# zhoubin-me/agent0

Hardware: AMD Instinct MI355X
Metric: env-frames/sec (learner FPS: transitions collected and saved to replay per second with the learner running, pre-frameskip) (higher is better)
Workload: dtype f32

## Files before the change

agent0_amd/csrc/igemm_x9.h:

```cpp
#pragma once
#include "igemm.h"
#if defined(__HIPCC__)
#include <hip/hip_ext.h>
#endif

#if defined(__HIPCC__)

typedef __bf16 a0_bf16x8g __attribute__((ext_vector_type(8)));
typedef short a0_s16x4 __attribute__((ext_vector_type(4)));
typedef uint32_t a0_u32x2g __attribute__((ext_vector_type(2)));
typedef uint32_t a0_u32x4g __attribute__((ext_vector_type(4)));

struct a0_x9_piece {
    a0_f4 v;
    uint32_t h[4], m[4], l[4];
    A0_D void split(int e) {
        const float x = e == 0 ? v.x : e == 1 ? v.y : e == 2 ? v.z : v.w;
        h[e] = __float_as_uint(x);
        const float r1 = x - __uint_as_float(h[e] & 0xffff0000u);
        m[e] = __float_as_uint(r1);
        const float r2 = r1 - __uint_as_float(m[e] & 0xffff0000u);
        l[e] = __float_as_uint(r2);
    }
    A0_D void pack(a0_u32x2g& hi, a0_u32x2g& mid, a0_u32x2g& lo) const {
// ... 119 lines not shown
        return v;
    }
};
template <int BX, int NTH, int KS> struct a0_x9_stager<OpPlanesKC, BX, NTH, KS, A0_KC> {
    static constexpr bool PRESPLIT = true;
    static constexpr int TPR = 4 * KS;
    static constexpr int RPP = NTH / TPR;
    static constexpr int R = BX / RPP;
    static_assert(BX % RPP == 0, "tile rows per pass");
    typedef a0_x9_image<A0_KC, BX, KS> IM;
    typedef OpPlanesKC OP;
    OP::Row rows[R];
    OP::KInfo ki;
    struct Slot { OP::Raw raw[R]; unsigned okmask; };
    A0_D void init(const OP::Params& P, int x0, int X, int kb, int ke, int tid) {
#pragma unroll
        for (int j = 0; j < R; ++j) rows[j] = OP::row(P, x0 + tid / TPR + RPP * j, X);
        ki = OP::kinfo(P, kb + 4 * (tid % TPR), ke);
    }
    template <bool FULL = false> A0_D void fetch_piece(const OP::Params& P, Slot& s, int j, int k0, int ke, int tid) {
        s.raw[j] = OP::load(P, rows[j], ki);
        if (j == R - 1) ki = OP::kinfo(P, k0 + 16 * KS + 4 * (tid % TPR), ke);
    }
    template <bool RS, bool FULL = false> A0_D a0_f4 value(const Slot&, int, a0_f4&) const { return a0_zero4(); }
    A0_D void store(const a0_x9_piece&, int, char*, int) const {}
    A0_D void store_raw(const Slot& s, int j, char* lds, int tid) const {
        const int r = tid / TPR + RPP * j;
        char* p = lds + r * IM::PITCH + 8 * (tid % TPR);
        a0_u32x2g hi, mid; hi.x = s.raw[j].a.x; hi.y = s.raw[j].a.y; mid.x = s.raw[j].a.z; mid.y = s.raw[j].a.w;
        *(a0_u32x2g*)(p) = hi;
        *(a0_u32x2g*)(p + IM::PLANE) = mid;
        *(a0_u32x2g*)(p + 2 * IM::PLANE) = s.raw[j].b;
    }
    A0_D static int frag_base(int lane, int woff) { return (woff + (lane & 31)) * IM::PITCH + (lane >> 5) * 16; }
    A0_D static a0_u32x4g frag(const char* plane, int base, int blk, int s) {
        return *(const a0_u32x4g*)(plane + base + blk * 32 * IM::PITCH + s * 32);
    }
};

template <class OA, class OB, int WM, int WN, int MT, int NT, int KS = 2> struct a0_x9_geom {
    static constexpr int BX = WM * MT * 32, BY = WN * NT * 32;
    static constexpr int ABYTES = 3 * a0_x9_image<OA::MODE, BX, KS>::PLANE;
    static constexpr int BBYTES = 3 * a0_x9_image<OB::MODE, BY, KS>::PLANE;
    static constexpr int LDS_BYTES = 2 * (ABYTES + BBYTES);
};

template <class OP> struct a0_x9_plain { static constexpr bool value = false; };
template <> struct a0_x9_plain<OpMatKC> { static constexpr bool value = true; };
template <> struct a0_x9_plain<OpMatXC> { static constexpr bool value = true; };
struct OpPlanesKC;
template <> struct a0_x9_plain<OpPlanesKC> { static constexpr bool value = true; };
template <class EP> struct a0_is_hadamard { static constexpr bool value = false; };
template <> struct a0_is_hadamard<EpiHadamard> { static constexpr bool value = true; };

int a0_x9_products_now();
template <class OA, class OB, class EP, int WM, int WN, int MT, int NT, int KS = 2, int NPR = 9, bool FULL = false>
__device__ __forceinline__ void a0_igemm_x9_body(const typename OA::Params& pa, const typename OB::Params& pb,
                                                 const typename EP::Params& pe, int X, int Y, int K, int kchunk, int gx, int gy) {
    static_assert(WM * WN == 4 || WM * WN == 8, "four or eight waves per workgroup");
    static_assert(KS == 1 || KS == 2, "tiles of 16 or 32 k");
    typedef a0_x9_geom<OA, OB, WM, WN, MT, NT, KS> G;
    constexpr int BK = 16 * KS, BX = G::BX, BY = G::BY, NTH = WM * WN * 64;
    typedef a0_x9_stager<OA, BX, NTH, KS> SA;
    typedef a0_x9_stager<OB, BY, NTH, KS> SB;
    constexpr int APL = a0_x9_image<OA::MODE, BX, KS>::PLANE, BPL = a0_x9_image<OB::MODE, BY, KS>::PLANE;
    constexpr int RA = SA::R, RB = SB::R, NP = RA + RB;
    static_assert(NPR == 9 || NPR == 6, "nine or six cross products");
    constexpr int NG = NPR * KS;
    static_assert(!EP::ROWSUM_A || OA::MODE == A0_XC, "row sums need an x-contiguous A operand");
    extern __shared__ __attribute__((aligned(16))) char a0_x9_lds[];
    char* const As = a0_x9_lds;
    char* const Bs = a0_x9_lds + 2 * G::ABYTES;

    const int tid = threadIdx.x, lane = tid & 63, wave = tid >> 6;
    const int wm = wave / WN, wn = wave % WN;
    int bx, by, bz;
    {
        const int n = gridDim.x, id = blockIdx.x, per = n >> 3;
        const int L = (id < (per << 3)) ? (id & 7) * per + (id >> 3) : id;
        if (gy <= gx) { by = L % gy; const int t = L / gy; bx = t % gx; bz = t / gx; }
        else          { bx = L % gx; const int t = L / gx; by = t % gy; bz = t / gy; }
    }
    const int x0 = bx * BX, y0 = by * BY;
    const int kb = bz * kchunk;
    const int ke = (K < kb + kchunk) ? K : (kb + kchunk);

    SA sa; SB sb;
    sa.init(pa, x0, X, kb, ke, tid);
    sb.init(pb, y0, Y, kb, ke, tid);

    a0_acc16 acc[MT][NT];
#pragma unroll
    for (int i = 0; i < MT; ++i)
#pragma unroll
        for (int j = 0; j < NT; ++j)
#pragma unroll
            for (int r = 0; r < 16; ++r) acc[i][j][r] = 0.f;

    a0_f4 rowsum = a0_zero4();

    auto fetch_piece = [&](typename SA::Slot& s_a, typename SB::Slot& s_b, int p, int k0) {
        if (p < RA) sa.template fetch_piece<FULL>(pa, s_a, p, k0, ke, tid);
        else sb.template fetch_piece<FULL>(pb, s_b, p - RA, k0, ke, tid);
    };
    a0_x9_piece pc;
    auto micro = [&](int u, const typename SA::Slot& s_a_c, const typename SB::Slot& s_b_c, typename SA::Slot& s_a, typename SB::Slot& s_b,
// ... 70 lines not shown
        __syncthreads();
    }
    if constexpr (EP::ROWSUM_A) {
        if (by == 0) {
            constexpr int Q = BX / 4;
            a0_f4* red = (a0_f4*)a0_x9_lds;
            red[tid] = rowsum;
            __syncthreads();
            if (tid < BX && x0 + tid < X) {
                const float* rf = (const float*)a0_x9_lds;
                float t = 0.f;
#pragma unroll
                for (int g = 0; g < NTH / Q; ++g) t += rf[4 * (g * Q + (tid >> 2)) + (tid & 3)];
                EP::store_rowsum(pe, x0 + tid, t, bz);
            }
        }
    }

    if constexpr (a0_is_hadamard<EP>::value) {
        static_assert(MT == 2, "EpiHadamard: waves of 64 rows");
#pragma unroll
        for (int j = 0; j < NT; ++j) {
            const int y = y0 + wn * (NT * 32) + j * 32 + (lane & 31);
            const bool yok = y < Y;
            const int yy = yok ? y : 0;
            float s64 = 0.f;
#pragma unroll
            for (int i = 0; i < MT; ++i) {
                const int xb = x0 + wm * (MT * 32) + i * 32;
                const int bsmp = xb / pe.n;
                const float f = pe.feat[(long long)bsmp * pe.ld + yy];
                float sacc = 0.f;
                float ev[16];
#pragma unroll
                for (int r = 0; r < 16; ++r) ev[r] = pe.emb[(long long)(xb + (r & 3) + 8 * (r >> 2) + 4 * (lane >> 5)) * pe.ld + yy];
#pragma unroll
                for (int r = 0; r < 16; ++r) {
                    const long long idx = (long long)(xb + (r & 3) + 8 * (r >> 2) + 4 * (lane >> 5)) * pe.ld + yy;
                    const float g = acc[i][j][r];
                    if (yok) pe.demb[idx] = (ev[r] > 0.f) ? g * f : 0.f;
                    sacc += g * ev[r];
                }
                sacc += __shfl_xor(sacc, 32, 64);
                if (pe.n == 32) { if (yok && lane < 32) pe.d3[(long long)bsmp * pe.ld + y] = (f > 0.f) ? sacc : 0.f; }
                else {
                    s64 += sacc;
                    if (i == MT - 1 && yok && lane < 32) pe.d3[(long long)bsmp * pe.ld + y] = (f > 0.f) ? s64 : 0.f;
                }
            }
        }
        return;
    }
    const int z = bz;
#pragma unroll
    for (int i = 0; i < MT; ++i)
#pragma unroll
        for (int j = 0; j < NT; ++j) {
            const int y = y0 + wn * (NT * 32) + j * 32 + (lane & 31);
#pragma unroll
            for (int r = 0; r < 16; ++r) {
                const int x = x0 + wm * (MT * 32) + i * 32 + (r & 3) + 8 * (r >> 2) + 4 * (lane >> 5);
                if (x < X && y < Y) EP::store(pe, x, y, acc[i][j][r], z);
            }
        }
}

template <class OA, class OB, class EP, int WM, int WN, int MT, int NT, int KS = 2, int NPR = 9, bool FULL = false>
__global__ __launch_bounds__(WM * WN * 64) void a0_igemm_x9_kernel(typename OA::Params pa, typename OB::Params pb,
                                                           typename EP::Params pe, int X, int Y, int K, int kchunk, int gx, int gy) {
    a0_igemm_x9_body<OA, OB, EP, WM, WN, MT, NT, KS, NPR, FULL>(pa, pb, pe, X, Y, K, kchunk, gx, gy);
}

template <class OA, class OB, class EP> struct a0_x9_group { typename OA::Params pa[3]; typename OB::Params pb[3]; typename EP::Params pe[3]; };
template <class OA, class OB, class EP, int WM, int WN, int MT, int NT, int KS = 2, int NPR = 9>
__global__ __launch_bounds__(WM * WN * 64) void a0_igemm_x9_group_kernel(a0_x9_group<OA, OB, EP> G, int X, int Y, int K, int kchunk, int gx, int gy) {
    const int g = blockIdx.y;
    a0_igemm_x9_body<OA, OB, EP, WM, WN, MT, NT, KS, NPR>(G.pa[g], G.pb[g], G.pe[g], X, Y, K, kchunk, gx, gy);
}

template <class OA, class OB, class EP, int WM, int WN, int MT, int NT, int KS = 2>
static inline hipError_t a0_igemm_x9_group_launch(hipStream_t st, int n, const a0_x9_group<OA, OB, EP>& grp, int X, int Y, int K, int splits, hipEvent_t ev0 = nullptr,
                                                  hipEvent_t ev1 = nullptr) {
    typedef a0_x9_geom<OA, OB, WM, WN, MT, NT, KS> G;
    const int six = a0_x9_products_now() == 6;
    auto kern = six ? a0_igemm_x9_group_kernel<OA, OB, EP, WM, WN, MT, NT, KS, 6> : a0_igemm_x9_group_kernel<OA, OB, EP, WM, WN, MT, NT, KS, 9>;
    static bool configured[2] = {false, false};
    if (!configured[six]) {
        hipError_t e = hipFuncSetAttribute((const void*)kern, hipFuncAttributeMaxDynamicSharedMemorySize, G::LDS_BYTES);
        if (e != hipSuccess) return e;
        configured[six] = true;
    }
    if (splits < 1) splits = 1;
    constexpr int BK = 16 * KS;
    const int ktiles = (K + BK - 1) / BK;
    const int kchunk = ((ktiles + splits - 1) / splits) * BK;
    const int gx = (X + G::BX - 1) / G::BX, gy = (Y + G::BY - 1) / G::BY;
    if (ev0) hipExtLaunchKernelGGL(kern, dim3((unsigned)(gx * gy * splits), (unsigned)n), dim3(WM * WN * 64), (uint32_t)G::LDS_BYTES, st, ev0, ev1, 0, grp, X, Y, K, kchunk, gx, gy);
    else hipLaunchKernelGGL(kern, dim3((unsigned)(gx * gy * splits), (unsigned)n), dim3(WM * WN * 64), G::LDS_BYTES, st, grp, X, Y, K, kchunk, gx, gy);
    return hipGetLastError();
}

template <class OA1, class OB1, class EP1, class OA2, class OB2, class EP2, int WM, int WN, int MT, int NT, int KS = 2, int NPR = 9>
__global__ __launch_bounds__(WM * WN * 64) void a0_igemm_x9_pair_kernel(typename OA1::Params pa1, typename OB1::Params pb1, typename EP1::Params pe1, int X1, int Y1, int K1, int kc1,
                                                                int gx1, int gy1, typename OA2::Params pa2, typename OB2::Params pb2, typename EP2::Params pe2, int X2, int Y2,
                                                                int K2, int kc2, int gx2, int gy2) {
    const int n = gridDim.x, id = blockIdx.x, per = n >> 3;
    const int L = (id < (per << 3)) ? (id & 7) * per + (id >> 3) : id;
    if (blockIdx.y == 0) { if (L < gx1 * gy1) a0_igemm_x9_body<OA1, OB1, EP1, WM, WN, MT, NT, KS, NPR>(pa1, pb1, pe1, X1, Y1, K1, kc1, gx1, gy1); }
    else if (L < gx2 * gy2) a0_igemm_x9_body<OA2, OB2, EP2, WM, WN, MT, NT, KS, NPR>(pa2, pb2, pe2, X2, Y2, K2, kc2, gx2, gy2);
}

template <class OA1, class OB1, class EP1, class OA2, class OB2, class EP2, int WM, int WN, int MT, int NT, int KS = 2>
static inline hipError_t a0_igemm_x9_pair_launch(hipStream_t st, const typename OA1::Params& pa1, const typename OB1::Params& pb1, const typename EP1::Params& pe1, int X1, int Y1, int K1,
                                                 const typename OA2::Params& pa2, const typename OB2::Params& pb2, const typename EP2::Params& pe2, int X2, int Y2, int K2) {
    typedef a0_x9_geom<OA1, OB1, WM, WN, MT, NT, KS> G1;
    typedef a0_x9_geom<OA2, OB2, WM, WN, MT, NT, KS> G2;
    constexpr int LDS = G1::LDS_BYTES > G2::LDS_BYTES ? G1::LDS_BYTES : G2::LDS_BYTES;
    const int six = a0_x9_products_now() == 6;
    auto kern = six ? a0_igemm_x9_pair_kernel<OA1, OB1, EP1, OA2, OB2, EP2, WM, WN, MT, NT, KS, 6> : a0_igemm_x9_pair_kernel<OA1, OB1, EP1, OA2, OB2, EP2, WM, WN, MT, NT, KS, 9>;
    static bool configured[2] = {false, false};
    if (!configured[six]) {
        hipError_t e = hipFuncSetAttribute((const void*)kern, hipFuncAttributeMaxDynamicSharedMemorySize, LDS);
        if (e != hipSuccess) return e;
        configured[six] = true;
    }
    constexpr int BK = 16 * KS;
    const int kc1 = ((K1 + BK - 1) / BK) * BK, kc2 = ((K2 + BK - 1) / BK) * BK;
    const int gx1 = (X1 + G1::BX - 1) / G1::BX, gy1 = (Y1 + G1::BY - 1) / G1::BY, gx2 = (X2 + G2::BX - 1) / G2::BX, gy2 = (Y2 + G2::BY - 1) / G2::BY;
    const int gmax = gx1 * gy1 > gx2 * gy2 ? gx1 * gy1 : gx2 * gy2;
    hipLaunchKernelGGL(kern, dim3((unsigned)gmax, 2), dim3(WM * WN * 64), LDS, st, pa1, pb1, pe1, X1, Y1, K1, kc1, gx1, gy1, pa2, pb2, pe2, X2, Y2, K2, kc2, gx2, gy2);
    return hipGetLastError();
}

template <class OA1, class OB1, class EP1, class OA2, class OB2, class EP2, int WM, int WN, int MT, int NT, int KS = 2, int NPR = 9>
__global__ __launch_bounds__(WM * WN * 64) void a0_igemm_x9_trio_kernel(typename OA1::Params pa1, typename OB1::Params pb1, typename EP1::Params pe1, int X1, int Y1, int K1, int kc1,
                                                                int gx1, int gy1, typename OA2::Params pa2, typename OB2::Params pb2, typename EP2::Params pe2, int X2, int Y2,
                                                                int K2, int kc2, int gx2, int gy2, typename OA2::Params pa3, typename OB2::Params pb3, typename EP2::Params pe3,
                                                                int X3, int Y3, int K3, int kc3, int gx3, int gy3) {
    if (blockIdx.y == 1) a0_igemm_x9_body<OA1, OB1, EP1, WM, WN, MT, NT, KS, NPR>(pa1, pb1, pe1, X1, Y1, K1, kc1, gx1, gy1);
    else if (blockIdx.y == 2) a0_igemm_x9_body<OA2, OB2, EP2, WM, WN, MT, NT, KS, NPR>(pa2, pb2, pe2, X2, Y2, K2, kc2, gx2, gy2);
    else {
        const int n = gridDim.x, id = blockIdx.x, per = n >> 3;
        const int L = (id < (per << 3)) ? (id & 7) * per + (id >> 3) : id;
        if (L >= gx3 * gy3) return;
        a0_igemm_x9_body<OA2, OB2, EP2, WM, WN, MT, NT, KS, NPR>(pa3, pb3, pe3, X3, Y3, K3, kc3, gx3, gy3);
    }
}

template <class OA1, class OB1, class EP1, class OA2, class OB2, class EP2, int WM, int WN, int MT, int NT, int KS = 2>
static inline hipError_t a0_igemm_x9_trio_launch(hipStream_t st, const typename OA1::Params& pa1, const typename OB1::Params& pb1, const typename EP1::Params& pe1, int X1, int Y1, int K1,
                                                 const typename OA2::Params& pa2, const typename OB2::Params& pb2, const typename EP2::Params& pe2, int X2, int Y2, int K2,
                                                 const typename OA2::Params& pa3, const typename OB2::Params& pb3, const typename EP2::Params& pe3, int X3, int Y3, int K3) {
    typedef a0_x9_geom<OA1, OB1, WM, WN, MT, NT, KS> G1;
    typedef a0_x9_geom<OA2, OB2, WM, WN, MT, NT, KS> G2;
    constexpr int LDS = G1::LDS_BYTES > G2::LDS_BYTES ? G1::LDS_BYTES : G2::LDS_BYTES;
    const int six = a0_x9_products_now() == 6;
    auto kern = six ? a0_igemm_x9_trio_kernel<OA1, OB1, EP1, OA2, OB2, EP2, WM, WN, MT, NT, KS, 6> : a0_igemm_x9_trio_kernel<OA1, OB1, EP1, OA2, OB2, EP2, WM, WN, MT, NT, KS, 9>;
    static bool configured[2] = {false, false};
    if (!configured[six]) {
        hipError_t e = hipFuncSetAttribute((const void*)kern, hipFuncAttributeMaxDynamicSharedMemorySize, LDS);
        if (e != hipSuccess) return e;
        configured[six] = true;
    }
    constexpr int BK = 16 * KS;
    const int kc1 = ((K1 + BK - 1) / BK) * BK, kc2 = ((K2 + BK - 1) / BK) * BK, kc3 = ((K3 + BK - 1) / BK) * BK;
    const int gx1 = (X1 + G1::BX - 1) / G1::BX, gy1 = (Y1 + G1::BY - 1) / G1::BY, gx2 = (X2 + G2::BX - 1) / G2::BX, gy2 = (Y2 + G2::BY - 1) / G2::BY;
    const int gx3 = (X3 + G2::BX - 1) / G2::BX, gy3 = (Y3 + G2::BY - 1) / G2::BY;
    if (gx1 * gy1 != gx2 * gy2 || gx3 * gy3 > gx1 * gy1) return hipErrorInvalidValue;
    hipLaunchKernelGGL(kern, dim3((unsigned)(gx1 * gy1), 3), dim3(WM * WN * 64), LDS, st, pa1, pb1, pe1, X1, Y1, K1, kc1, gx1, gy1, pa2, pb2, pe2, X2, Y2, K2, kc2, gx2, gy2,
                       pa3, pb3, pe3, X3, Y3, K3, kc3, gx3, gy3);
    return hipGetLastError();
}

template <class OA, class OB, class EP, int WM, int WN, int MT, int NT, int KS = 2>
static inline hipError_t a0_igemm_x9_launch(hipStream_t st, const typename OA::Params& pa, const typename OB::Params& pb,
                                            const typename EP::Params& pe, int X, int Y, int K, int splits, hipEvent_t ev0 = nullptr, hipEvent_t ev1 = nullptr) {
    typedef a0_x9_geom<OA, OB, WM, WN, MT, NT, KS> G;
    if (splits < 1) splits = 1;
    constexpr int BK = 16 * KS;
    constexpr bool can_full = a0_x9_plain<OA>::value && a0_x9_plain<OB>::value && !EP::ROWSUM_A;
    const int six = a0_x9_products_now() == 6;
    const int full = (can_full && (K % BK) == 0) ? 1 : 0;
    typedef void (*a0_kern_t)(typename OA::Params, typename OB::Params, typename EP::Params, int, int, int, int, int, int);
    a0_kern_t kern;
    if constexpr (can_full) kern = full ? (six ? (a0_kern_t)a0_igemm_x9_kernel<OA, OB, EP, WM, WN, MT, NT, KS, 6, true> : (a0_kern_t)a0_igemm_x9_kernel<OA, OB, EP, WM, WN, MT, NT, KS, 9, true>)
                                        : (six ? (a0_kern_t)a0_igemm_x9_kernel<OA, OB, EP, WM, WN, MT, NT, KS, 6> : (a0_kern_t)a0_igemm_x9_kernel<OA, OB, EP, WM, WN, MT, NT, KS, 9>);
    else kern = six ? (a0_kern_t)a0_igemm_x9_kernel<OA, OB, EP, WM, WN, MT, NT, KS, 6> : (a0_kern_t)a0_igemm_x9_kernel<OA, OB, EP, WM, WN, MT, NT, KS, 9>;
    static bool configured[4] = {false, false, false, false};
    if (!configured[2 * full + six]) {
        hipError_t e = hipFuncSetAttribute((const void*)kern, hipFuncAttributeMaxDynamicSharedMemorySize, G::LDS_BYTES);
        if (e != hipSuccess) return e;
        configured[2 * full + six] = true;
    }
    const int ktiles = (K + BK - 1) / BK;
    const int kchunk = ((ktiles + splits - 1) / splits) * BK;
    const int gx = (X + G::BX - 1) / G::BX, gy = (Y + G::BY - 1) / G::BY;
    if (ev0) hipExtLaunchKernelGGL(kern, dim3((unsigned)(gx * gy * splits)), dim3(WM * WN * 64), (uint32_t)G::LDS_BYTES, st, ev0, ev1, 0, pa, pb, pe, X, Y, K, kchunk, gx, gy);
    else hipLaunchKernelGGL(kern, dim3((unsigned)(gx * gy * splits)), dim3(WM * WN * 64), G::LDS_BYTES, st, pa, pb, pe, X, Y, K, kchunk, gx, gy);
    return hipGetLastError();
}

template <class OP> struct a0_x9_ok { static constexpr bool value = sizeof(typename OP::Raw) == sizeof(a0_f4); };

#endif
```

agent0_amd/csrc/loss.hip:

```cpp
#include "a0_internal.h"
#include "actor_tail.h"

__global__ void a0_dueling_fwd_kernel(const float* __restrict__ raw, int ld, float* __restrict__ q, int R, int A, int T, int dueling) {
    long long i = (long long)blockIdx.x * blockDim.x + threadIdx.x;
    if (i >= (long long)R * T) return;
    const int r = (int)(i / T), t = (int)(i % T);
    const float* x = raw + (long long)r * ld;
    float* o = q + (long long)r * A * T;
    if (!dueling) {
        for (int a = 0; a < A; ++a) o[a * T + t] = x[a * T + t];
        return;
    }
    float s = 0.f;
    for (int a = 0; a < A; ++a) s += x[a * T + t];
    const float mean = s / (float)A;
    const float v = x[A * T + t];
    for (int a = 0; a < A; ++a) o[a * T + t] = v + (x[a * T + t] - mean);
}

__global__ void a0_dueling_bwd_kernel(const float* __restrict__ dq, float* __restrict__ draw, int ld, int R, int A, int T, int dueling) {
    long long i = (long long)blockIdx.x * blockDim.x + threadIdx.x;
    if (i >= (long long)R * ld) return;
    const int r = (int)(i / ld), c = (int)(i % ld);
    const float* g = dq + (long long)r * A * T;
// ... 424 lines not shown
        if (c < A) {
            out = (c == ab) ? g : 0.f;
            if (dueling) {
                float s = 0.f;
                for (int a = 0; a < A; ++a) s += (a == ab) ? g : 0.f;
                out -= s / (float)A;
            }
        } else if (dueling && c == A) {
            float s = 0.f;
            for (int a = 0; a < A; ++a) s += (a == ab) ? g : 0.f;
            out = s;
        }
        o[c] = out;
    }
}

extern "C" int a0_dqn_head_loss(const float* h_on, const float* h_tg, const float* h_sel, const float* W_on, const float* b_on, const float* W_tg,
                                const float* b_tg, int A, int dueling, int ld, const int* act, const float* rew, const float* done, const float* wgt,
                                float gamma_n, int B, float* loss, float* q_on_out, float* q_tg_out, float* draw, int* nan_flag, void* stream) {
    const int NQ = A + (dueling ? 1 : 0);
    if (!h_on || !h_tg || !W_on || !b_on || !W_tg || !b_tg || !act || !rew || !done || !wgt || !loss || !q_on_out || !draw || !nan_flag || B < 1 || A < 1 || NQ > 24 ||
        ld < NQ)
        return a0_fail(A0_EINVAL, "a0_dqn_head_loss: bad argument (A + dueling <= 24)");
    const size_t lds = (size_t)2 * NQ * 512 * sizeof(float);
    static size_t configured = 0;
    if (lds > configured) {
        if (hipFuncSetAttribute((const void*)a0_dqn_head_loss_kernel, hipFuncAttributeMaxDynamicSharedMemorySize, (int)lds) != hipSuccess)
            return a0_fail(A0_EINVAL, "a0_dqn_head_loss: LDS");
        configured = lds;
    }
    hipLaunchKernelGGL(a0_dqn_head_loss_kernel, dim3((B + 3) / 4), dim3(256), lds, (hipStream_t)stream, h_on, h_tg, h_sel, W_on, b_on, W_tg, b_tg, A, dueling, ld, act,
                       rew, done, wgt, gamma_n, B, loss, q_on_out, q_tg_out, draw, nan_flag);
    return a0_fail_hip((int)hipGetLastError(), "a0_dqn_head_loss");
}

struct a0_mdqn_par { float tau, lo; float* q_sel_out; };
template <class QN, class QC>
A0_D float a0_mdqn_target(QN qn, QC qc, int A, int a, float rew, float done, float gamma_n, float tau, float lo);
template <bool MDQN>
__global__ __launch_bounds__(256) void a0_dqn_head_loss_slabs_kernel(const float* __restrict__ s_on, const float* __restrict__ s_tg, const float* __restrict__ s_sel,
                                                                     long long slab_stride, int nslab, const float* __restrict__ b1_on,
                                                                     const float* __restrict__ b1_tg, float* __restrict__ h_on_out,
                                                                     const float* __restrict__ W_on, const float* __restrict__ b_on, const float* __restrict__ W_tg,
                                                                     const float* __restrict__ b_tg, int A, int dueling, int ld, const int* __restrict__ act,
                                                                     const float* __restrict__ rew, const float* __restrict__ done, const float* __restrict__ wgt,
                                                                     float gamma_n, int B, float* __restrict__ loss, float* __restrict__ q_on_out,
                                                                     float* __restrict__ q_tg_out, float* __restrict__ draw, int* __restrict__ nan_flag,
                                                                     float* __restrict__ dh_out, a0_mdqn_par M) {
    extern __shared__ float wsm[];
    __shared__ float raw[4][3][32];
    __shared__ float dsh[4][32];
    const int lane = threadIdx.x & 63, wave = threadIdx.x >> 6;
    const int NQ = A + (dueling ? 1 : 0);
    for (int i = threadIdx.x; i < NQ * 128; i += 256) { ((a0_f4*)wsm)[i] = ((const a0_f4*)W_on)[i]; ((a0_f4*)wsm)[NQ * 128 + i] = ((const a0_f4*)W_tg)[i]; }
    const int b = blockIdx.x * 4 + wave;
    const int br = b < B ? b : B - 1;
    float ho[8], ht[8], hs[8];
#pragma unroll
    for (int i = 0; i < 8; ++i) { ho[i] = 0.f; ht[i] = 0.f; hs[i] = 0.f; }
    const long long ro = (long long)br * 512 + lane;
    auto sum4 = [&](const float* __restrict__ sp, float (&h)[8]) {
        int z = 0;
        for (; z + 4 <= nslab; z += 4) {
            float t[4][8];
#pragma unroll
            for (int zz = 0; zz < 4; ++zz)
#pragma unroll
                for (int i = 0; i < 8; ++i) t[zz][i] = sp[(long long)(z + zz) * slab_stride + ro + 64 * i];
#pragma unroll
            for (int zz = 0; zz < 4; ++zz)
#pragma unroll
                for (int i = 0; i < 8; ++i) h[i] += t[zz][i];
        }
        for (; z < nslab; ++z) {
            float t[8];
#pragma unroll
            for (int i = 0; i < 8; ++i) t[i] = sp[(long long)z * slab_stride + ro + 64 * i];
#pragma unroll
            for (int i = 0; i < 8; ++i) h[i] += t[i];
        }
    };
    sum4(s_on, ho);
    sum4(s_tg, ht);
    if (s_sel) sum4(s_sel, hs);
#pragma unroll
    for (int i = 0; i < 8; ++i) {
        const float bo = b1_on[lane + 64 * i], bt = b1_tg[lane + 64 * i];
        float v = ho[i] + bo; ho[i] = v < 0.f ? 0.f : v;
        v = ht[i] + bt; ht[i] = v < 0.f ? 0.f : v;
        v = hs[i] + (MDQN ? bt : bo); hs[i] = v < 0.f ? 0.f : v;
    }
    __syncthreads();
    if (b >= B) return;
#pragma unroll
    for (int i = 0; i < 8; ++i) h_on_out[(long long)b * 512 + lane + 64 * i] = ho[i];
    for (int a = 0; a < NQ; ++a) {
        const float* wo = wsm + a * 512;
        const float* wt = wsm + (NQ + a) * 512;
        float so = 0.f, st = 0.f, ss = 0.f;
#pragma unroll
        for (int i = 0; i < 8; ++i) {
            const float w1 = wo[lane + 64 * i], w2 = wt[lane + 64 * i];
            so = fmaf(ho[i], w1, so);
            ss = fmaf(hs[i], MDQN ? w2 : w1, ss);
            st = fmaf(ht[i], w2, st);
        }
        so = a0_wave_sum(so); st = a0_wave_sum(st); ss = a0_wave_sum(ss);
        if (lane == 0) { raw[wave][0][a] = so + b_on[a]; raw[wave][1][a] = st + b_tg[a]; raw[wave][2][a] = ss + (MDQN ? b_tg[a] : b_on[a]); }
    }
    if (lane == 0) {
    const int nsel = (s_sel && !MDQN) ? 2 : 1;
    float mean[3] = {0.f, 0.f, 0.f}, v[3] = {0.f, 0.f, 0.f};
    if (dueling)
        for (int s3 = 0; s3 < 3; ++s3) {
            float t = 0.f;
            for (int a = 0; a < A; ++a) t += raw[wave][s3][a];
            mean[s3] = t / (float)A;
            v[s3] = raw[wave][s3][A];
        }
    auto q = [&](int s3, int a) { return dueling ? v[s3] + (raw[wave][s3][a] - mean[s3]) : raw[wave][s3][a]; };
    float best = 0.f;
    int a_star = 0;
    for (int a = 0; a < A; ++a) {
        const float x = q(nsel, a);
        if (a == 0 || x > best) { best = x; a_star = a; }
        q_on_out[(long long)b * A + a] = q(0, a);
        if (q_tg_out) q_tg_out[(long long)b * A + a] = q(1, a);
        if (MDQN && M.q_sel_out) M.q_sel_out[(long long)b * A + a] = q(2, a);
    }
    const int ab = act[b];
    float y;
    if (MDQN) {
        y = a0_mdqn_target([&](int k) { return q(1, k); }, [&](int k) { return q(2, k); }, A, ab, rew[b], done[b], gamma_n, M.tau, M.lo);
    } else {
        const float qn = q(1, a_star);
        y = rew[b] + (gamma_n * (1.f - done[b])) * qn;
    }
    const float d = q(0, ab) - y;
    const float ad = fabsf(d);
    const float l = (ad < 1.f) ? 0.5f * d * d : ad - 0.5f;
    loss[b] = l;
    if (l != l) atomicOr(nan_flag, 1);
    const float g = wgt[b] * fminf(fmaxf(d, -1.f), 1.f);
    float* o = draw + (long long)b * ld;
    for (int c = 0; c < ld; ++c) {
        float out = 0.f;
        if (c < A) {
            out = (c == ab) ? g : 0.f;
            if (dueling) {
                float s = 0.f;
                for (int a = 0; a < A; ++a) s += (a == ab) ? g : 0.f;
                out -= s / (float)A;
            }
        } else if (dueling && c == A) {
            float s = 0.f;
            for (int a = 0; a < A; ++a) s += (a == ab) ? g : 0.f;
            out = s;
        }
        o[c] = out;
        if (c < 32) dsh[wave][c] = out;
    }
    }
    if (dh_out) {
        __builtin_amdgcn_s_waitcnt(0xc07f);
        __builtin_amdgcn_wave_barrier();
#pragma unroll
        for (int i = 0; i < 8; ++i) {
            float acc = 0.f;
            for (int c = 0; c < NQ; ++c) acc = fmaf(dsh[wave][c], wsm[c * 512 + lane + 64 * i], acc);
            dh_out[(long long)b * 512 + lane + 64 * i] = ho[i] > 0.f ? acc : 0.f;
        }
    }
}

extern "C" int a0_dqn_head_loss_slabs(const float* slabs_on, const float* slabs_tg, const float* slabs_sel, long long slab_stride, int nslab, const float* b1_on,
                                      const float* b1_tg, float* h_on_out, const float* W_on, const float* b_on, const float* W_tg, const float* b_tg, int A,
                                      int dueling, int ld, const int* act, const float* rew, const float* done, const float* wgt, float gamma_n, int B, float* loss,
                                      float* q_on_out, float* q_tg_out, float* draw, int* nan_flag, float* dh_out, void* stream) {
    const int NQ = A + (dueling ? 1 : 0);
    if (!slabs_on || !slabs_tg || !b1_on || !b1_tg || !h_on_out || !W_on || !b_on || !W_tg || !b_tg || !act || !rew || !done || !wgt || !loss || !q_on_out || !draw ||
        !nan_flag || B < 1 || A < 1 || NQ > 24 || ld < NQ || nslab < 1 || slab_stride < (long long)B * 512)
        return a0_fail(A0_EINVAL, "a0_dqn_head_loss_slabs: bad argument (A + dueling <= 24)");
    const size_t lds = (size_t)2 * NQ * 512 * sizeof(float);
    static size_t configured = 0;
    if (lds > configured) {
        if (hipFuncSetAttribute((const void*)a0_dqn_head_loss_slabs_kernel<false>, hipFuncAttributeMaxDynamicSharedMemorySize, (int)lds) != hipSuccess)
            return a0_fail(A0_EINVAL, "a0_dqn_head_loss_slabs: LDS");
        configured = lds;
    }
    hipLaunchKernelGGL(a0_dqn_head_loss_slabs_kernel<false>, dim3((B + 3) / 4), dim3(256), lds, (hipStream_t)stream, slabs_on, slabs_tg, slabs_sel, slab_stride, nslab, b1_on, b1_tg,
                       h_on_out, W_on, b_on, W_tg, b_tg, A, dueling, ld, act, rew, done, wgt, gamma_n, B, loss, q_on_out, q_tg_out, draw, nan_flag, dh_out, a0_mdqn_par{0.f, 0.f, nullptr});
    return a0_fail_hip((int)hipGetLastError(), "a0_dqn_head_loss_slabs");
}

extern "C" int a0_mdqn_head_loss_slabs(const float* slabs_on, const float* slabs_tg, const float* slabs_cur, long long slab_stride, int nslab, const float* b1_on,
                                       const float* b1_tg, float* h_on_out, const float* W_on, const float* b_on, const float* W_tg, const float* b_tg, int A,
// ... 534 lines not shown
```

agent0_amd/csrc/net.hip:

```cpp
#include "igemm_x9.h"
#include "short_k_fwd.h"
#include "a0_internal.h"
#include "net_impl.h"
#include "update_tail.h"

#include <vector>

__global__ __launch_bounds__(256) void a0_reduce_slabs_kernel(const float* __restrict__ slabs, long long slab_stride, int nslab,
                                                               float* __restrict__ out, long long count) {
    __shared__ float red[8][33];
    const int c = threadIdx.x & 31, g = threadIdx.x >> 5;
    const long long i = (long long)blockIdx.x * 32 + c;
    float s = 0.f;
    if (i < count)
        for (int z = g; z < nslab; z += 8) s += slabs[(long long)z * slab_stride + i];
    red[g][c] = s;
    __syncthreads();
    if (g == 0 && i < count) {
        float t = 0.f;
#pragma unroll
        for (int j = 0; j < 8; ++j) t += red[j][c];
        out[i] = t;
    }
}
// ... 668 lines not shown
extern "C" int a0_actor_qhead_env_step_enc(const float* feat, int E, int K, const float* W1, const float* b1, const float* W2, const float* b2, int A, int dueling,
                                           float* scratch, unsigned long long seed, unsigned int stream_a, unsigned int stream_u, unsigned long long off_a,
                                           unsigned long long off_u, float eps, const long long* ctrl, const float* eps_ptr, int* action, float* qmax,
                                           unsigned long long env_seed, unsigned int rank, unsigned int g, const uint8_t* obs_in, uint8_t* obs_out, float* ep_ret,
                                           float* final_mask, float* final_ret, int n, long long steps, double gamma, int* ring_act, float* ring_rew, float* ring_done,
                                           const uint8_t* obs0, uint8_t* frames, long long cap, long long start_slot, int* r_act, float* r_rew, float* r_done, int task,
                                           const float* wt, const a0_encoder_weights* w, float* act3_next, void* stream) {
    return a0_actor_qhead_env_step_enc_wp(feat, E, K, W1, b1, W2, b2, A, dueling, scratch, seed, stream_a, stream_u, off_a, off_u, eps, ctrl, eps_ptr, action, qmax, env_seed, rank, g, obs_in, obs_out, ep_ret, final_mask, final_ret, n, steps, gamma, ring_act, ring_rew, ring_done, obs0, frames, cap, start_slot, r_act, r_rew, r_done, task, wt, w, act3_next, nullptr, stream);
}

__global__ __launch_bounds__(256) void a0_mean_rows_kernel(const float* __restrict__ x, int E, float* __restrict__ out) {
    __shared__ float red[256];
    const float* p = x + (long long)blockIdx.x * E;
    float s = 0.f;
    for (int e = threadIdx.x; e < E; e += 256) s += p[e];
    red[threadIdx.x] = s;
    __syncthreads();
    for (int o = 128; o > 0; o >>= 1) { if ((int)threadIdx.x < o) red[threadIdx.x] += red[threadIdx.x + o]; __syncthreads(); }
    if (threadIdx.x == 0) out[blockIdx.x] = red[0] / (float)E;
}

extern "C" int a0_mean_rows(const float* x, int T, int E, float* out, void* stream) {
    if (!x || !out || T < 1 || E < 1) return a0_fail(A0_EINVAL, "a0_mean_rows: bad argument");
    hipLaunchKernelGGL(a0_mean_rows_kernel, dim3(T), dim3(256), 0, (hipStream_t)stream, x, E, out);
    return a0_fail_hip((int)hipGetLastError(), "a0_mean_rows");
}

extern "C" int a0_dense_dgrad(const float* dY, const float* W, const float* act_mask, float* dX, int R, int N, int K, void* stream) {
    A0_TRY
    if (!dY || !W || !dX || R < 1 || (N & 3) || (K & 3)) return a0_fail(A0_EINVAL, "a0_dense_dgrad: bad shape");
    a0_hip_backend bk{(hipStream_t)stream};
    a0_dense_dgrad_impl(bk, dY, W, act_mask, dX, R, N, K);
    return A0_OK;
    A0_CATCH
}

extern "C" int a0_dense_dgrad_hadamard_ok(int R, int N, int K, int n) {
    return (g_gemm_x9 != 0 && (n == 32 || n == 64) && R >= 4096 && !(R & 255) && !(R % n) && !(N & 15) && N >= 64 && !(K & 3) && K >= 128) ? 1 : 0;
}
extern "C" int a0_dense_dgrad_hadamard(const float* dY, const float* W, const float* emb, const float* feat, float* demb, float* d3, int R, int N, int K, int n, void* stream) {
    A0_TRY
    if (!dY || !W || !emb || !feat || !demb || !d3 || !a0_dense_dgrad_hadamard_ok(R, N, K, n)) return a0_fail(A0_EINVAL, "a0_dense_dgrad_hadamard: shapes a0_dense_dgrad_hadamard_ok accepts");
    const a0_mat_src a{dY, N};
    const a0_mat_src bw{W, K};
    const EpiHadamard::Params e{emb, feat, demb, d3, K, n};
    hipEvent_t e0 = nullptr, e1 = nullptr;
    const bool probe = a0_probe_events(A0_TAG_DENSE_DGRAD, &e0, &e1);
    A0_HIP_THROW((a0_igemm_x9_launch<OpMatKC, OpMatXC, EpiHadamard, 4, 2, 2, 2, 1>((hipStream_t)stream, a, bw, e, R, K, N, 1, e0, e1)));
    if (probe) a0_probe_commit(2.0 * (double)R * (double)N * (double)K);
    return A0_OK;
    A0_CATCH
}

extern "C" int a0_dense_dgrad_wgrad_ok(int R, int N, int K) {
    const long long b128 = (long long)((R + 127) / 128) * ((K + 63) / 64), b64 = (long long)((N + 63) / 64) * ((K + 63) / 64);
    return (g_gemm_x9 != 0 && g_probe.tag == 0 && R == N && R >= 1 && R <= 1024 && !(N & 3) && !(K & 3) && b128 < 256 && b64 >= 256 && N >= 512 &&
            (long long)((R + 127) / 128) * ((K + 127) / 128) < A0_X9_BIG_TILES) ? 1 : 0;
}
static int a0_dense_dgrad_wgrad_small_ok(int R, int N, int K) {
    const long long t1 = (long long)((R + 63) / 64) * ((K + 63) / 64), t2 = (long long)((N + 63) / 64) * ((K + 63) / 64);
    return (g_gemm_x9 != 0 && g_probe.tag == 0 && R >= 64 && R <= 1024 && N >= 64 && !(N & 3) && !(K & 3) && t1 + t2 <= 256 && t2 >= 16) ? 1 : 0;
}
extern "C" int a0_dense_dgrad_wgrad_ok2(int R, int N, int K) { return (a0_dense_dgrad_wgrad_ok(R, N, K) || a0_dense_dgrad_wgrad_small_ok(R, N, K)) ? 1 : 0; }
extern "C" int a0_dense_dgrad_wgrad(const float* dY, const float* W, const float* X, int ldx, float* dX, float* grad, int R, int N, int K, void* stream) {
    A0_TRY
    if (!dY || !W || !X || !dX || !grad || ldx < K || (ldx & 3) || !a0_dense_dgrad_wgrad_ok2(R, N, K)) return a0_fail(A0_EINVAL, "a0_dense_dgrad_wgrad: shapes a0_dense_dgrad_wgrad_ok2 accepts");
    a0_mat_src a1{dY, N}, b1{W, K};
    EpiMaskMat::Params e1{dX, X, K};
    a0_mat_src a2{dY, N}, b2{X, ldx};
    EpiWgradSlab::Params e2{grad, 0, K, (long long)N * K};
    if (!a0_dense_dgrad_wgrad_ok(R, N, K)) {
        A0_HIP_THROW((a0_igemm_x9_pair_launch<OpMatKC, OpMatXC, EpiMaskMat, OpMatXC, OpMatXC, EpiWgradSlab, 2, 2, 1, 1>((hipStream_t)stream, a1, b1, e1, R, K, N, a2, b2, e2, N, K, R)));
        return A0_OK;
    }
    A0_HIP_THROW((a0_igemm_x9_pair_launch<OpMatKC, OpMatXC, EpiMaskMat, OpMatXC, OpMatXC, EpiWgradSlab, 4, 2, 1, 1>((hipStream_t)stream, a1, b1, e1, R, K, N, a2, b2, e2, N, K, R)));
    return A0_OK;
    A0_CATCH
}

extern "C" int a0_dense_dgrad_wgrad2_ok(int R, int N, int K, int N2, int K2) {
    return (a0_dense_dgrad_wgrad_ok(R, N, K) && N2 >= 4 && !(N2 & 3) && K2 >= 4 && !(K2 & 3) &&
            (long long)((N2 + 127) / 128) * ((K2 + 63) / 64) <= 8) ? 1 : 0;
}
extern "C" int a0_dense_dgrad_wgrad2(const float* dY, const float* W, const float* X, int ldx, float* dX, float* grad, int R, int N, int K,
                                     const float* dY2, const float* X2, int ldx2, float* grad2, int N2, int K2, void* stream) {
    A0_TRY
    if (!dY || !W || !X || !dX || !grad || ldx < K || (ldx & 3) || !a0_dense_dgrad_wgrad_ok(R, N, K)) return a0_fail(A0_EINVAL, "a0_dense_dgrad_wgrad2: shapes a0_dense_dgrad_wgrad_ok accepts");
    if (!dY2 || !X2 || !grad2 || N2 < 4 || (N2 & 3) || K2 < 4 || (K2 & 3) || ldx2 < K2 || (ldx2 & 3) ||
        (long long)((N2 + 127) / 128) * ((K2 + 63) / 64) > (long long)((R + 127) / 128) * ((K + 63) / 64))
        return a0_fail(A0_EINVAL, "a0_dense_dgrad_wgrad2: the second layer's weight gradient must have no more 128 x 64 tiles than the first layer's data gradient");
    a0_mat_src a1{dY, N}, b1{W, K};
    EpiMaskMat::Params e1{dX, X, K};
    a0_mat_src a2{dY, N}, b2{X, ldx};
    EpiWgradSlab::Params e2{grad, 0, K, (long long)N * K};
    a0_mat_src a3{dY2, N2}, b3{X2, ldx2};
    EpiWgradSlab::Params e3{grad2, 0, K2, (long long)N2 * K2};
    A0_HIP_THROW((a0_igemm_x9_trio_launch<OpMatKC, OpMatXC, EpiMaskMat, OpMatXC, OpMatXC, EpiWgradSlab, 4, 2, 1, 1>((hipStream_t)stream, a1, b1, e1, R, K, N, a2, b2, e2, N, K, R,
                                                                                                                  a3, b3, e3, N2, K2, R)));
    return A0_OK;
    A0_CATCH
}

extern "C" long long a0_dense_wgrad_scratch(int R, int N, int K) { return a0_dense_wgrad_scratch_impl(R, N, K); }

extern "C" int a0_dense_wgrad(const float* dY, const float* X, int ldx, float* grad, int R, int N, int K, float* slabs, void* stream) {
    A0_TRY
    if (!dY || !X || !grad || R < 1 || (N & 3) || (K & 3) || (ldx & 3)) return a0_fail(A0_EINVAL, "a0_dense_wgrad: bad shape");
    if (a0_dense_wgrad_scratch_impl(R, N, K) > 0 && !slabs) return a0_fail(A0_EINVAL, "a0_dense_wgrad: needs slab scratch");
    a0_hip_backend bk{(hipStream_t)stream};
    a0_dense_wgrad_impl(bk, dY, X, ldx, grad, R, N, K, slabs);
    return A0_OK;
    A0_CATCH
}

extern "C" int a0_dense_wgrad_multi(int n, const float* const* dY, const float* const* X, const int* ldx, float* const* grad, const int* R, const int* N, const int* K,
                                    float* slabs, const long long* slab_off, a0_pending_reduce* pend, void* stream) {
    A0_TRY
    if (n < 1 || n > 4 || !dY || !X || !ldx || !grad || !R || !N || !K || !slab_off) return a0_fail(A0_EINVAL, "a0_dense_wgrad_multi: 1..4 layers");
    a0_hip_backend bk{(hipStream_t)stream};
    a0_reduce_seg segs[4];
    int nseg = 0;
    for (int i = 0; i < n; ++i) {
        if (!dY[i] || !X[i] || !grad[i] || R[i] < 1 || (N[i] & 3) || (K[i] & 3) || (ldx[i] & 3)) return a0_fail(A0_EINVAL, "a0_dense_wgrad_multi: bad shape");
        if (a0_dense_wgrad_scratch_impl(R[i], N[i], K[i]) > 0 && !slabs) return a0_fail(A0_EINVAL, "a0_dense_wgrad_multi: needs slab scratch");
        a0_reduce_seg seg;
        a0_dense_wgrad_impl(bk, dY[i], X[i], ldx[i], grad[i], R[i], N[i], K[i], slabs ? slabs + slab_off[i] : nullptr, &seg);
        if (seg.nslab > 0) segs[nseg++] = seg;
    }
    if (pend) {
        if (pend->n < 0 || pend->n + nseg > 4) return a0_fail(A0_EINVAL, "a0_dense_wgrad_multi: more than four pending reductions");
        for (int k = 0; k < nseg; ++k) pend->seg[pend->n++] = segs[k];
    } else if (nseg > 0) bk.reduce_segments(segs, nseg);
    return A0_OK;
    A0_CATCH
}

extern "C" int a0_net_encoder_wgrad(const a0_net* n, const a0_encoder_weights* w, const a0_frames_arg* f, int B, const float* act1, const float* act2,
                                    const float* d3, const float* d2, const float* d1, float* g1, float* g2, float* g3, float* slabs, const a0_pending_reduce* pend,
                                    void* stream) {
    A0_TRY
    if (!n || !w || !f || !f->frames || !act1 || !act2 || !d3 || !d2 || !d1 || !g1 || !g2 || !g3 || B < 1) return a0_fail(A0_EINVAL, "a0_net_encoder_wgrad: null argument");
    if (a0_encoder_bwd_scratch_impl(n->core, B) > 0 && !slabs) return a0_fail(A0_EINVAL, "a0_net_encoder_wgrad: needs slab scratch");
    if (pend && (pend->n < 0 || pend->n > 4)) return a0_fail(A0_EINVAL, "a0_net_encoder_wgrad: bad pending reductions");
    a0_hip_backend bk{(hipStream_t)stream};
    a0_encoder_bwd_impl(bk, n->core, *w, *f, B, act1, act2, d3, const_cast<float*>(d2), const_cast<float*>(d1), g1, g2, g3, slabs, false, pend);
    return A0_OK;
    A0_CATCH
}

__global__ void a0_tail_prep_kernel(a0_tail_prep P) {
// ... 37 lines not shown
```

agent0_amd/csrc/operands.h:

```cpp
#pragma once
#include "a0_defs.h"

enum { A0_KC = 0, A0_XC = 1 };

struct a0_frames_src {
    const uint8_t* frames;
    const int* slot;
    a0_geom g;
    int chan_off;
    const a0_i4* ktab;
    int aligned4;
};

A0_HD uint32_t a0_u8x4_load(const uint8_t* p, int aligned4) {
    if (aligned4) return *(const uint32_t*)p;
    return (uint32_t)p[0] | ((uint32_t)p[1] << 8) | ((uint32_t)p[2] << 16) | ((uint32_t)p[3] << 24);
}

A0_HD float a0_div255(float x) {
    const float r = 1.0f / 255.0f;
    const float q0 = x * r;
#if defined(__HIPCC__)
    const float e = __builtin_fmaf(-q0, 255.0f, x);
    return __builtin_fmaf(e, r, q0);
// ... 168 lines not shown
        P.out[(long long)x * P.ld + y] = v;
    }
};

struct EpiBiasActMul {
    static constexpr bool ROWSUM_A = false;
    struct Params { float* out; const float* bias; int ld; int relu; const float* mul; int group; unsigned group_magic; };
    A0_HD static void store(const Params& P, int x, int y, float v, int) {
        v += P.bias[y];
        if (P.relu) v = (v < 0.f) ? 0.f : v;
        const int g = a0_udiv(x, P.group, P.group_magic);
        P.out[(long long)x * P.ld + y] = v * P.mul[(long long)g * P.ld + y];
    }
};

struct EpiSlab {
    static constexpr bool ROWSUM_A = false;
    struct Params { float* out; long long slab_stride; int ld; };
    A0_HD static void store(const Params& P, int x, int y, float v, int z) {
        P.out[(long long)z * P.slab_stride + (long long)x * P.ld + y] = v;
    }
};

struct EpiDgrad {
    static constexpr bool ROWSUM_A = false;
    struct Params {
        float* dx; const float* act;
        int HWv, Wv;
        int Hfull, Wfull, C;
        int s, ph, pw;
        long long sample_stride;
    };
    A0_HD static void store(const Params& P, int x, int y, float v, int) {
        int b = x / P.HWv;
        int rem = x - b * P.HWv;
        int h2 = rem / P.Wv;
        int w2 = rem - h2 * P.Wv;
        int h = h2 * P.s + P.ph, w = w2 * P.s + P.pw;
        if (h >= P.Hfull || w >= P.Wfull) return;
        long long i = (long long)b * P.sample_stride + ((long long)h * P.Wfull + w) * P.C + y;
        P.dx[i] = (P.act[i] > 0.f) ? v : 0.f;
    }
};

struct EpiHadamard {
    static constexpr bool ROWSUM_A = false;
    struct Params { const float* emb; const float* feat; float* demb; float* d3; int ld; int n; };
    A0_HD static void store(const Params&, int, int, float, int) {}
};

struct EpiMaskMat {
    static constexpr bool ROWSUM_A = false;
    struct Params { float* dx; const float* act; int ld; };
    A0_HD static void store(const Params& P, int x, int y, float v, int) {
        long long i = (long long)x * P.ld + y;
        P.dx[i] = (P.act[i] > 0.f) ? v : 0.f;
    }
};
```

Before: 2.378 million.

## Batch mask loads in masked epilogue, widen fc1 GEMM tiles, prefetch loss-kernel inputs

Three changes go in together. The masked dgrad epilogue now loads every activation mask value before any store, so those loads can overlap. The fused fc1 dgrad/wgrad pair and trio kernels use 1x2 wave tiles (128x128 blocks) in place of 1x1, and the second-layer eligibility check is relaxed to match. The dueling loss kernel issues its first four slab loads and the bias and per-sample scalar loads before the weight copy into LDS, and reads per-action biases through readlane. The aim is to hide global-memory latency and reduce the block count, at the cost of more registers and fewer workgroups for small shapes.

```diff
diff --git a/agent0_amd/csrc/igemm_x9.h b/agent0_amd/csrc/igemm_x9.h
--- a/agent0_amd/csrc/igemm_x9.h
+++ b/agent0_amd/csrc/igemm_x9.h
@@ -195,6 +195,8 @@
 template <> struct a0_x9_plain<OpPlanesKC> { static constexpr bool value = true; };
 template <class EP> struct a0_is_hadamard { static constexpr bool value = false; };
 template <> struct a0_is_hadamard<EpiHadamard> { static constexpr bool value = true; };
+template <class EP> struct a0_is_masked { static constexpr bool value = false; };
+template <> struct a0_is_masked<EpiMaskMat> { static constexpr bool value = true; };
 
 int a0_x9_products_now();
 template <class OA, class OB, class EP, int WM, int WN, int MT, int NT, int KS = 2, int NPR = 9, bool FULL = false>
@@ -371,6 +373,32 @@
         return;
     }
     const int z = bz;
+    if constexpr (a0_is_masked<EP>::value) {
+        float mk[MT][NT][16];
+#pragma unroll
+        for (int i = 0; i < MT; ++i)
+#pragma unroll
+            for (int j = 0; j < NT; ++j) {
+                const int y = y0 + wn * (NT * 32) + j * 32 + (lane & 31);
+#pragma unroll
+                for (int r = 0; r < 16; ++r) {
+                    const int x = x0 + wm * (MT * 32) + i * 32 + (r & 3) + 8 * (r >> 2) + 4 * (lane >> 5);
+                    mk[i][j][r] = EP::mask(pe, x < X ? x : X - 1, y < Y ? y : Y - 1);
+                }
+            }
+#pragma unroll
+        for (int i = 0; i < MT; ++i)
+#pragma unroll
+            for (int j = 0; j < NT; ++j) {
+                const int y = y0 + wn * (NT * 32) + j * 32 + (lane & 31);
+#pragma unroll
+                for (int r = 0; r < 16; ++r) {
+                    const int x = x0 + wm * (MT * 32) + i * 32 + (r & 3) + 8 * (r >> 2) + 4 * (lane >> 5);
+                    if (x < X && y < Y) EP::store_masked(pe, x, y, acc[i][j][r], mk[i][j][r]);
+                }
+            }
+        return;
+    }
 #pragma unroll
     for (int i = 0; i < MT; ++i)
 #pragma unroll
@@ -435,6 +463,7 @@
     typedef a0_x9_geom<OA1, OB1, WM, WN, MT, NT, KS> G1;
     typedef a0_x9_geom<OA2, OB2, WM, WN, MT, NT, KS> G2;
     constexpr int LDS = G1::LDS_BYTES > G2::LDS_BYTES ? G1::LDS_BYTES : G2::LDS_BYTES;
+    static_assert(LDS <= 160 * 1024, "a workgroup's tile buffers must fit the 160 KB of LDS");
     const int six = a0_x9_products_now() == 6;
     auto kern = six ? a0_igemm_x9_pair_kernel<OA1, OB1, EP1, OA2, OB2, EP2, WM, WN, MT, NT, KS, 6> : a0_igemm_x9_pair_kernel<OA1, OB1, EP1, OA2, OB2, EP2, WM, WN, MT, NT, KS, 9>;
     static bool configured[2] = {false, false};
@@ -473,6 +502,7 @@
     typedef a0_x9_geom<OA1, OB1, WM, WN, MT, NT, KS> G1;
     typedef a0_x9_geom<OA2, OB2, WM, WN, MT, NT, KS> G2;
     constexpr int LDS = G1::LDS_BYTES > G2::LDS_BYTES ? G1::LDS_BYTES : G2::LDS_BYTES;
+    static_assert(LDS <= 160 * 1024, "a workgroup's tile buffers must fit the 160 KB of LDS");
     const int six = a0_x9_products_now() == 6;
     auto kern = six ? a0_igemm_x9_trio_kernel<OA1, OB1, EP1, OA2, OB2, EP2, WM, WN, MT, NT, KS, 6> : a0_igemm_x9_trio_kernel<OA1, OB1, EP1, OA2, OB2, EP2, WM, WN, MT, NT, KS, 9>;
     static bool configured[2] = {false, false};
diff --git a/agent0_amd/csrc/loss.hip b/agent0_amd/csrc/loss.hip
--- a/agent0_amd/csrc/loss.hip
+++ b/agent0_amd/csrc/loss.hip
@@ -500,15 +500,19 @@
     __shared__ float dsh[4][32];
     const int lane = threadIdx.x & 63, wave = threadIdx.x >> 6;
     const int NQ = A + (dueling ? 1 : 0);
-    for (int i = threadIdx.x; i < NQ * 128; i += 256) { ((a0_f4*)wsm)[i] = ((const a0_f4*)W_on)[i]; ((a0_f4*)wsm)[NQ * 128 + i] = ((const a0_f4*)W_tg)[i]; }
     const int b = blockIdx.x * 4 + wave;
     const int br = b < B ? b : B - 1;
+    const int ab = act[br];
+    const float rew_b = rew[br], done_b = done[br], wgt_b = wgt[br];
+    const float hb_on = lane < NQ ? b_on[lane] : 0.f, hb_tg = lane < NQ ? b_tg[lane] : 0.f;
+    float b1o[8], b1t[8];
+#pragma unroll
+    for (int i = 0; i < 8; ++i) { b1o[i] = b1_on[lane + 64 * i]; b1t[i] = b1_tg[lane + 64 * i]; }
     float ho[8], ht[8], hs[8];
 #pragma unroll
     for (int i = 0; i < 8; ++i) { ho[i] = 0.f; ht[i] = 0.f; hs[i] = 0.f; }
     const long long ro = (long long)br * 512 + lane;
-    auto sum4 = [&](const float* __restrict__ sp, float (&h)[8]) {
-        int z = 0;
+    auto sum4 = [&](const float* __restrict__ sp, float (&h)[8], int z) {
         for (; z + 4 <= nslab; z += 4) {
             float t[4][8];
 #pragma unroll
@@ -528,12 +532,42 @@
             for (int i = 0; i < 8; ++i) h[i] += t[i];
         }
     };
-    sum4(s_on, ho);
-    sum4(s_tg, ht);
-    if (s_sel) sum4(s_sel, hs);
+    const int z0 = nslab >= 4 ? 4 : 0;
+    float t_on[4][8], t_tg[4][8], t_sel[4][8];
+    if (z0) {
+#pragma unroll
+        for (int zz = 0; zz < 4; ++zz)
+#pragma unroll
+            for (int i = 0; i < 8; ++i) {
+                t_on[zz][i] = s_on[(long long)zz * slab_stride + ro + 64 * i];
+                t_tg[zz][i] = s_tg[(long long)zz * slab_stride + ro + 64 * i];
+            }
+        if (s_sel) {
+#pragma unroll
+            for (int zz = 0; zz < 4; ++zz)
+#pragma unroll
+                for (int i = 0; i < 8; ++i) t_sel[zz][i] = s_sel[(long long)zz * slab_stride + ro + 64 * i];
+        }
+    }
+    for (int i = threadIdx.x; i < NQ * 128; i += 256) { ((a0_f4*)wsm)[i] = ((const a0_f4*)W_on)[i]; ((a0_f4*)wsm)[NQ * 128 + i] = ((const a0_f4*)W_tg)[i]; }
+    if (z0) {
+#pragma unroll
+        for (int zz = 0; zz < 4; ++zz)
+#pragma unroll
+            for (int i = 0; i < 8; ++i) { ho[i] += t_on[zz][i]; ht[i] += t_tg[zz][i]; }
+        if (s_sel) {
+#pragma unroll
+            for (int zz = 0; zz < 4; ++zz)
+#pragma unroll
+                for (int i = 0; i < 8; ++i) hs[i] += t_sel[zz][i];
+        }
+    }
+    sum4(s_on, ho, z0);
+    sum4(s_tg, ht, z0);
+    if (s_sel) sum4(s_sel, hs, z0);
 #pragma unroll
     for (int i = 0; i < 8; ++i) {
-        const float bo = b1_on[lane + 64 * i], bt = b1_tg[lane + 64 * i];
+        const float bo = b1o[i], bt = b1t[i];
         float v = ho[i] + bo; ho[i] = v < 0.f ? 0.f : v;
         v = ht[i] + bt; ht[i] = v < 0.f ? 0.f : v;
         v = hs[i] + (MDQN ? bt : bo); hs[i] = v < 0.f ? 0.f : v;
@@ -554,7 +588,8 @@
             st = fmaf(ht[i], w2, st);
         }
         so = a0_wave_sum(so); st = a0_wave_sum(st); ss = a0_wave_sum(ss);
-        if (lane == 0) { raw[wave][0][a] = so + b_on[a]; raw[wave][1][a] = st + b_tg[a]; raw[wave][2][a] = ss + (MDQN ? b_tg[a] : b_on[a]); }
+        const float bo_a = __int_as_float(__builtin_amdgcn_readlane(__float_as_int(hb_on), a)), bt_a = __int_as_float(__builtin_amdgcn_readlane(__float_as_int(hb_tg), a));
+        if (lane == 0) { raw[wave][0][a] = so + bo_a; raw[wave][1][a] = st + bt_a; raw[wave][2][a] = ss + (MDQN ? bt_a : bo_a); }
     }
     if (lane == 0) {
     const int nsel = (s_sel && !MDQN) ? 2 : 1;
@@ -576,20 +611,19 @@
         if (q_tg_out) q_tg_out[(long long)b * A + a] = q(1, a);
         if (MDQN && M.q_sel_out) M.q_sel_out[(long long)b * A + a] = q(2, a);
     }
-    const int ab = act[b];
     float y;
     if (MDQN) {
-        y = a0_mdqn_target([&](int k) { return q(1, k); }, [&](int k) { return q(2, k); }, A, ab, rew[b], done[b], gamma_n, M.tau, M.lo);
+        y = a0_mdqn_target([&](int k) { return q(1, k); }, [&](int k) { return q(2, k); }, A, ab, rew_b, done_b, gamma_n, M.tau, M.lo);
     } else {
         const float qn = q(1, a_star);
-        y = rew[b] + (gamma_n * (1.f - done[b])) * qn;
+        y = rew_b + (gamma_n * (1.f - done_b)) * qn;
     }
     const float d = q(0, ab) - y;
     const float ad = fabsf(d);
     const float l = (ad < 1.f) ? 0.5f * d * d : ad - 0.5f;
     loss[b] = l;
     if (l != l) atomicOr(nan_flag, 1);
-    const float g = wgt[b] * fminf(fmaxf(d, -1.f), 1.f);
+    const float g = wgt_b * fminf(fmaxf(d, -1.f), 1.f);
     float* o = draw + (long long)b * ld;
     for (int c = 0; c < ld; ++c) {
         float out = 0.f;
diff --git a/agent0_amd/csrc/net.hip b/agent0_amd/csrc/net.hip
--- a/agent0_amd/csrc/net.hip
+++ b/agent0_amd/csrc/net.hip
@@ -744,6 +744,8 @@
     A0_CATCH
 }
 
+static constexpr int A0_FC1_MT = 1, A0_FC1_NT = 2;
+static constexpr int A0_FC1_BX = 128 * A0_FC1_MT, A0_FC1_BY = 64 * A0_FC1_NT;
 extern "C" int a0_dense_dgrad_wgrad_ok(int R, int N, int K) {
     const long long b128 = (long long)((R + 127) / 128) * ((K + 63) / 64), b64 = (long long)((N + 63) / 64) * ((K + 63) / 64);
     return (g_gemm_x9 != 0 && g_probe.tag == 0 && R == N && R >= 1 && R <= 1024 && !(N & 3) && !(K & 3) && b128 < 256 && b64 >= 256 && N >= 512 &&
@@ -765,29 +767,28 @@
         A0_HIP_THROW((a0_igemm_x9_pair_launch<OpMatKC, OpMatXC, EpiMaskMat, OpMatXC, OpMatXC, EpiWgradSlab, 2, 2, 1, 1>((hipStream_t)stream, a1, b1, e1, R, K, N, a2, b2, e2, N, K, R)));
         return A0_OK;
     }
-    A0_HIP_THROW((a0_igemm_x9_pair_launch<OpMatKC, OpMatXC, EpiMaskMat, OpMatXC, OpMatXC, EpiWgradSlab, 4, 2, 1, 1>((hipStream_t)stream, a1, b1, e1, R, K, N, a2, b2, e2, N, K, R)));
+    A0_HIP_THROW((a0_igemm_x9_pair_launch<OpMatKC, OpMatXC, EpiMaskMat, OpMatXC, OpMatXC, EpiWgradSlab, 4, 2, A0_FC1_MT, A0_FC1_NT>((hipStream_t)stream, a1, b1, e1, R, K, N, a2, b2, e2, N, K, R)));
     return A0_OK;
     A0_CATCH
 }
 
 extern "C" int a0_dense_dgrad_wgrad2_ok(int R, int N, int K, int N2, int K2) {
-    return (a0_dense_dgrad_wgrad_ok(R, N, K) && N2 >= 4 && !(N2 & 3) && K2 >= 4 && !(K2 & 3) &&
-            (long long)((N2 + 127) / 128) * ((K2 + 63) / 64) <= 8) ? 1 : 0;
+    return (a0_dense_dgrad_wgrad_ok(R, N, K) && N2 >= 4 && !(N2 & 3) && N2 <= 128 && K2 >= 4 && !(K2 & 3) && K2 <= 512) ? 1 : 0;
 }
 extern "C" int a0_dense_dgrad_wgrad2(const float* dY, const float* W, const float* X, int ldx, float* dX, float* grad, int R, int N, int K,
                                      const float* dY2, const float* X2, int ldx2, float* grad2, int N2, int K2, void* stream) {
     A0_TRY
     if (!dY || !W || !X || !dX || !grad || ldx < K || (ldx & 3) || !a0_dense_dgrad_wgrad_ok(R, N, K)) return a0_fail(A0_EINVAL, "a0_dense_dgrad_wgrad2: shapes a0_dense_dgrad_wgrad_ok accepts");
     if (!dY2 || !X2 || !grad2 || N2 < 4 || (N2 & 3) || K2 < 4 || (K2 & 3) || ldx2 < K2 || (ldx2 & 3) ||
-        (long long)((N2 + 127) / 128) * ((K2 + 63) / 64) > (long long)((R + 127) / 128) * ((K + 63) / 64))
-        return a0_fail(A0_EINVAL, "a0_dense_dgrad_wgrad2: the second layer's weight gradient must have no more 128 x 64 tiles than the first layer's data gradient");
+        (long long)((N2 + A0_FC1_BX - 1) / A0_FC1_BX) * ((K2 + A0_FC1_BY - 1) / A0_FC1_BY) > (long long)((R + A0_FC1_BX - 1) / A0_FC1_BX) * ((K + A0_FC1_BY - 1) / A0_FC1_BY))
+        return a0_fail(A0_EINVAL, "a0_dense_dgrad_wgrad2: the second layer's weight gradient must have no more tiles than the first layer's data gradient");
     a0_mat_src a1{dY, N}, b1{W, K};
     EpiMaskMat::Params e1{dX, X, K};
     a0_mat_src a2{dY, N}, b2{X, ldx};
     EpiWgradSlab::Params e2{grad, 0, K, (long long)N * K};
     a0_mat_src a3{dY2, N2}, b3{X2, ldx2};
     EpiWgradSlab::Params e3{grad2, 0, K2, (long long)N2 * K2};
-    A0_HIP_THROW((a0_igemm_x9_trio_launch<OpMatKC, OpMatXC, EpiMaskMat, OpMatXC, OpMatXC, EpiWgradSlab, 4, 2, 1, 1>((hipStream_t)stream, a1, b1, e1, R, K, N, a2, b2, e2, N, K, R,
+    A0_HIP_THROW((a0_igemm_x9_trio_launch<OpMatKC, OpMatXC, EpiMaskMat, OpMatXC, OpMatXC, EpiWgradSlab, 4, 2, A0_FC1_MT, A0_FC1_NT>((hipStream_t)stream, a1, b1, e1, R, K, N, a2, b2, e2, N, K, R,
                                                                                                                   a3, b3, e3, N2, K2, R)));
     return A0_OK;
     A0_CATCH
diff --git a/agent0_amd/csrc/operands.h b/agent0_amd/csrc/operands.h
--- a/agent0_amd/csrc/operands.h
+++ b/agent0_amd/csrc/operands.h
@@ -244,8 +244,7 @@
 struct EpiMaskMat {
     static constexpr bool ROWSUM_A = false;
     struct Params { float* dx; const float* act; int ld; };
-    A0_HD static void store(const Params& P, int x, int y, float v, int) {
-        long long i = (long long)x * P.ld + y;
-        P.dx[i] = (P.act[i] > 0.f) ? v : 0.f;
-    }
-};
+    A0_HD static float mask(const Params& P, int x, int y) { return P.act[(long long)x * P.ld + y]; }
+    A0_HD static void store_masked(const Params& P, int x, int y, float v, float m) { P.dx[(long long)x * P.ld + y] = (m > 0.f) ? v : 0.f; }
+    A0_HD static void store(const Params& P, int x, int y, float v, int) { store_masked(P, x, y, v, mask(P, x, y)); }
+};
```

Result: faster. 2.452 million, median of 6 (+3.1%).
